# MeteoSwiss/topo-descriptors

Hardware: AMD Instinct MI355X
Metric: Mpixels/s (and % HBM roofline) per descriptor, 1/2/4/8 MI355X (higher is better)
Workload: dtype f32

## Files before the change

include/topo_amd.h:

```cpp
#ifndef TOPO_AMD_H
#define TOPO_AMD_H

#include <stddef.h>
#include <stdint.h>

#ifdef __cplusplus
extern "C" {
#endif

#define TOPO_AMD_OK 0
#define TOPO_AMD_EINVAL (-1)
#define TOPO_AMD_EHIP (-2)
#define TOPO_AMD_ENODEV (-3)
#define TOPO_AMD_ERCCL (-4)
#define TOPO_AMD_EUNSUP (-5)
#define TOPO_AMD_EEMPTY (-6)

#define TOPO_AMD_DESC_TPI 0
#define TOPO_AMD_DESC_STD 1
#define TOPO_AMD_DESC_GAUSS 2
#define TOPO_AMD_DESC_GRADIENT 3
#define TOPO_AMD_DESC_SOBEL 4
#define TOPO_AMD_DESC_SX 5
#define TOPO_AMD_DESC_VALLEY_RIDGE 6
// ... 44 lines not shown
int topo_amd_tpi_std_dev(const float* in, int in_rows, int in_row0, int gny, int nx, int size,
                         int out_row0, int out_rows, float* tpi_out, float* std_out);

int topo_amd_tpi_multi_dev(const float* in, int in_rows, int in_row0, int gny, int nx, int n_sizes,
                           const int32_t* sizes, int out_row0, int out_rows, float* const* tpi_outs);
int topo_amd_gaussian_dev(const float* in, int in_rows, int in_row0, int gny, int nx,
                          double sigma_y, double sigma_x, int out_row0, int out_rows,
                          float* out);

int topo_amd_sobel_dev(const float* in, int in_rows, int in_row0, int gny, int nx,
                       int out_row0, int out_rows, float* dx_out, float* dy_out);

int topo_amd_gradient_dev(const float* in, int in_rows, int in_row0, int gny, int nx,
                          double sigma, double sig_ratio, int res_mode, const void* res_x,
                          const void* res_y, int out_row0, int out_rows, float* dx_out,
                          float* dy_out, float* slope_out, float* aspect_out);

int topo_amd_sx_dev(const float* in, int in_rows, int in_row0, int gny, int nx,
                    const int32_t* dj, const int32_t* di, const double* dist, int n_off,
                    int window, double height, int out_row0, int out_rows, float* out);

int topo_amd_sx_multi_dev(const float* in, int in_rows, int in_row0, int gny, int nx, int n_az,
                          const int32_t* first, const int32_t* dj, const int32_t* di,
                          const double* dist, const int32_t* window, double height,
                          int out_row0, int out_rows, float* const* outs);

#define TOPO_AMD_VALLEY_MAX_PLANES 16
int topo_amd_valley_ridge_dev(const float* in, int in_rows, int in_row0, int gny, int nx,
                              const float* taps, const int32_t* ksize, const float* angles,
                              int n_angles, int n_planes, double mean, double stdev,
                              int out_row0, int out_rows, float* norm_out, float* dir_out);
int topo_amd_valley_route(int* route);
int topo_amd_tpi_route(int* route);
int topo_amd_mean_std_dev(const float* in, size_t count, double* mean, double* stdev);

int topo_amd_fill_na_dev(const float* in, int in_rows, int in_row0, int gny, int nx, const double* x_coords,
                         double min_elevation, int out_row0, int out_rows, float* out, uint8_t* missing_out);

int topo_amd_release_host_planes(void);
int topo_amd_host_chunks(int* chunks);
int topo_amd_tpi_f32(const float* dem, int ny, int nx, int size, double sigma, float* out);
int topo_amd_std_f32(const float* dem, int ny, int nx, int size, double sigma, float* out);
int topo_amd_tpi_std_f32(const float* dem, int ny, int nx, int size, double sigma,
                         float* tpi_out, float* std_out);
int topo_amd_tpi_std_multi_f32(const float* dem, int ny, int nx, int n_scales, const int32_t* sizes,
                               const double* sigmas, float* const* tpi_outs, float* const* std_outs);
int topo_amd_gauss_f32(const float* dem, int ny, int nx, double sigma_y, double sigma_x,
                       float* out);
int topo_amd_sobel_f32(const float* dem, int ny, int nx, float* dx_out, float* dy_out);
int topo_amd_fill_na_f32(const float* dem, int ny, int nx, const double* x_coords, double min_elevation, float* out,
                         uint8_t* missing_out);
int topo_amd_gradient_f32(const float* dem, int ny, int nx, double sigma, double sig_ratio,
                          int res_mode, const void* res_x, const void* res_y, float* dx_out,
                          float* dy_out, float* slope_out, float* aspect_out);
int topo_amd_sx_f32(const float* dem, int ny, int nx, const int32_t* dj, const int32_t* di,
                    const double* dist, int n_off, int window, double height, float* out);
int topo_amd_sx_multi_f32(const float* dem, int ny, int nx, int n_az, const int32_t* first,
                          const int32_t* dj, const int32_t* di, const double* dist,
                          const int32_t* window, double height, float* const* outs);
int topo_amd_valley_ridge_f32(const float* dem, int ny, int nx, const float* taps,
                              const int32_t* ksize, const float* angles, int n_angles,
                              int n_planes, double mean, double stdev, float* norm_out,
                              float* dir_out);

#define TOPO_AMD_F32 0
#define TOPO_AMD_I16 1
// ... 81 lines not shown
```

topo_descriptors_amd/_lib.py:

```python
import ctypes as C
import os
import threading

import numpy as np

HERE = os.path.dirname(os.path.abspath(__file__))
LIB_PATH = os.environ.get("TOPO_AMD_LIBRARY") or os.path.join(HERE, "libtopo_amd.so")

_f32p = C.POINTER(C.c_float)
_i32p = C.POINTER(C.c_int32)
_f64p = C.POINTER(C.c_double)
_vp = C.c_void_p


class Raster(C.Structure):
    _fields_ = [("data", C.c_void_p), ("dtype", C.c_int32), ("has_nodata", C.c_int32),
                ("scale", C.c_double), ("offset", C.c_double), ("nodata", C.c_double)]


_rp = C.POINTER(Raster)
F32, I16, U16, I32, U8, F64 = range(6)
SOURCE_DTYPES = {np.dtype(np.float32): F32, np.dtype(np.int16): I16, np.dtype(np.uint16): U16,
                 np.dtype(np.int32): I32, np.dtype(np.uint8): U8, np.dtype(np.float64): F64}

SIGNATURES = {
    "topo_amd_version": (C.c_char_p, []),
    "topo_amd_last_error": (C.c_char_p, []),
    "topo_amd_device_count": (C.c_int, []),
    "topo_amd_init": (C.c_int, [C.c_int]),
    "topo_amd_shutdown": (C.c_int, []),
    "topo_amd_device_name": (C.c_int, [C.c_char_p, C.c_int]),
    "topo_amd_malloc": (C.c_int, [C.POINTER(_vp), C.c_size_t]),
    "topo_amd_free": (C.c_int, [_vp]),
    "topo_amd_host_alloc": (C.c_int, [C.POINTER(C.c_void_p), C.c_size_t]),
    "topo_amd_host_free": (C.c_int, [C.c_void_p]),
    "topo_amd_memcpy_h2d": (C.c_int, [_vp, _vp, C.c_size_t]),
    "topo_amd_memcpy_d2h": (C.c_int, [_vp, _vp, C.c_size_t]),
    "topo_amd_memcpy_d2d": (C.c_int, [_vp, _vp, C.c_size_t]),
    "topo_amd_memset": (C.c_int, [_vp, C.c_int, C.c_size_t]),
    "topo_amd_sync": (C.c_int, []),
    "topo_amd_release_host_planes": (C.c_int, []),
    "topo_amd_host_chunks": (C.c_int, [_i32p]),
    "topo_amd_valley_route": (C.c_int, [_i32p]),
    "topo_amd_tpi_route": (C.c_int, [_i32p]),
    "topo_amd_dem_changed": (C.c_int, [_vp, C.c_size_t]),
    "topo_amd_raster_scan_dev": (C.c_int, [_vp, C.c_int, C.c_int, C.c_int, C.c_int, C.c_int, C.c_int,
                                           C.POINTER(C.c_uint64), _f32p]),
    "topo_amd_raster_class_from_scan": (C.c_int, [_vp, C.c_int, C.c_int, C.c_int, C.POINTER(C.c_uint64), _f32p]),
    "topo_amd_raster_class_set": (C.c_int, [_vp, C.c_int, C.c_int, C.c_int, C.c_int, C.c_float, C.c_float, C.c_float]),
    "topo_amd_raster_class_get": (C.c_int, [_vp, C.c_int, C.c_int, _i32p, _i32p, _f32p, _f32p, _f32p]),
    "topo_amd_shard_classify": (C.c_int, [_vp, C.c_int, C.c_int, C.c_int, C.c_int]),
    "topo_amd_timer_start": (C.c_int, []),
    "topo_amd_timer_stop": (C.c_int, [_f32p]),
    "topo_amd_mark": (C.c_int, [C.c_int]),
    "topo_amd_mark_elapsed": (C.c_int, [C.c_int, C.c_int, C.POINTER(C.c_float)]),
    "topo_amd_cu_count": (C.c_int, []),
    "topo_amd_synth_dem_dev": (C.c_int, [_vp, C.c_int, C.c_int, C.c_int, C.c_uint32, C.c_int]),
    "topo_amd_disc_tap_count": (C.c_int, [C.c_int]),
    "topo_amd_disc_mask": (C.c_int, [C.c_int, _f32p]),
    "topo_amd_halo_rows": (C.c_int, [C.c_int, C.c_double, C.c_double, _i32p, _i32p]),
    "topo_amd_tpi_std_dev": (C.c_int, [_vp, C.c_int, C.c_int, C.c_int, C.c_int, C.c_int, C.c_int,
                                       C.c_int, _vp, _vp]),
    "topo_amd_gaussian_dev": (C.c_int, [_vp, C.c_int, C.c_int, C.c_int, C.c_int, C.c_double,
                                        C.c_double, C.c_int, C.c_int, _vp]),
    "topo_amd_sobel_dev": (C.c_int, [_vp, C.c_int, C.c_int, C.c_int, C.c_int, C.c_int, C.c_int,
                                     _vp, _vp]),
    "topo_amd_gradient_dev": (C.c_int, [_vp, C.c_int, C.c_int, C.c_int, C.c_int, C.c_double,
                                        C.c_double, C.c_int, _vp, _vp, C.c_int, C.c_int, _vp, _vp,
                                        _vp, _vp]),
    "topo_amd_sx_dev": (C.c_int, [_vp, C.c_int, C.c_int, C.c_int, C.c_int, _i32p, _i32p, _f64p,
                                  C.c_int, C.c_int, C.c_double, C.c_int, C.c_int, _vp]),
    "topo_amd_tpi_multi_dev": (C.c_int, [_vp, C.c_int, C.c_int, C.c_int, C.c_int, C.c_int, _i32p, C.c_int, C.c_int,
                                         C.POINTER(_vp)]),
    "topo_amd_sx_multi_dev": (C.c_int, [_vp, C.c_int, C.c_int, C.c_int, C.c_int, C.c_int, _i32p, _i32p, _i32p,
                                        _f64p, _i32p, C.c_double, C.c_int, C.c_int, C.POINTER(_vp)]),
    "topo_amd_valley_ridge_dev": (C.c_int, [_vp, C.c_int, C.c_int, C.c_int, C.c_int, _vp, _i32p, _vp, C.c_int,
                                            C.c_int, C.c_double, C.c_double, C.c_int, C.c_int, _vp, _vp]),
# ... 160 lines not shown
```

topo_descriptors_amd/csrc/capi.hip:

```cpp
#include <rccl/rccl.h>

#include <algorithm>
#include <atomic>
#include <chrono>
#include <condition_variable>
#include <cmath>
#include <cstdio>
#include <cstdlib>
#include <cstring>
#include <map>
#include <mutex>

#include "common.hpp"
#include "decode.hpp"

#include <sys/mman.h>

#include <thread>

namespace topo {

static thread_local std::string g_error;

void set_error(const char* fmt, ...) {
// ... 940 lines not shown
    TOPO_REQUIRE(hptr != nullptr && bytes > 0, "host_alloc: bad arguments");
    TOPO_HIP(hipHostMalloc(hptr, bytes, hipHostMallocDefault));
    return TOPO_AMD_OK;
}
int topo_amd_host_free(void* hptr) {
    TOPO_ENTER();
    TOPO_TRY(require_ready());
    if (hptr) TOPO_HIP(hipHostFree(hptr));
    return TOPO_AMD_OK;
}

int topo_amd_release_host_planes(void) {
    TOPO_ENTER();
    TOPO_TRY(require_ready());
    Context& c = ctx();
    TOPO_HIP(hipStreamSynchronize(c.compute));
    for (size_t k = 0; k < c.host_planes.size(); ++k) {
        if (c.host_planes[k]) {
            dem_memo_forget(c.host_planes[k], c.host_plane_bytes[k]);
            TOPO_HIP(hipFree(c.host_planes[k]));
        }
    }
    c.host_planes.clear();
    c.host_plane_bytes.clear();
    return TOPO_AMD_OK;
}

int topo_amd_tpi_route(int* route) {
    TOPO_REQUIRE(route != nullptr, "tpi_route: NULL output");
    *route = t_tpi_route;
    return TOPO_AMD_OK;
}

int topo_amd_valley_route(int* route) {
    TOPO_REQUIRE(route != nullptr, "valley_route: NULL output");
    *route = t_valley_route;
    return TOPO_AMD_OK;
}

int topo_amd_host_chunks(int* chunks) {
    TOPO_REQUIRE(chunks != nullptr, "host_chunks: NULL output");
    *chunks = t_host_chunks;
    return TOPO_AMD_OK;
}

int topo_amd_memcpy_h2d(void* dst, const void* src, size_t bytes) {
    TOPO_ENTER();
    TOPO_TRY(require_ready());
    dem_memo_forget(dst, bytes);
    TOPO_HIP(hipMemcpyAsync(dst, src, bytes, hipMemcpyHostToDevice, ctx().compute));
    TOPO_HIP(hipStreamSynchronize(ctx().compute));
    return TOPO_AMD_OK;
}

int topo_amd_memcpy_d2h(void* dst, const void* src, size_t bytes) {
    TOPO_ENTER();
    TOPO_TRY(require_ready());
    {
        HostRun pages(false);
        pages.prefault(dst, bytes);
    }
    TOPO_HIP(hipMemcpyAsync(dst, src, bytes, hipMemcpyDeviceToHost, ctx().compute));
    TOPO_HIP(hipStreamSynchronize(ctx().compute));
    return check_gate_errors();
}

// ... 1215 lines not shown
    c.ghost = GhostGate();
    if (taken) return rc == TOPO_AMD_OK ? finish_gated(lean && device_gate, false) : rc;
    if (rc != TOPO_AMD_EUNSUP) return rc;
    return run_three(block, s, above, below, fn, true);
}


}
}

namespace {
int ensure_shard_class(const Shard& s) {
    if (s.rows_local == s.owned.gny || declared_class(s.owned, nullptr)) return TOPO_AMD_OK;
    return topo_amd_shard_classify(s.owned.in, s.rows_local, s.row0, s.owned.gny, s.owned.nx);
}
}

extern "C" {

int topo_amd_shard_tpi_std(float* block, int rows_local, int row0, int gny, int nx, int size,
                           float* tpi_out, float* std_out) {
    TOPO_ENTER();
    TOPO_TRY(require_ready());
    DiscRuns disc;
    TOPO_TRY(build_disc(size, &disc));
    const int above = -disc.dj_min, below = disc.dj_max;
    TOPO_TRY(shard_view(&block, above, below, "shard_tpi_std"));
    block += shard_view_offset(above, nx);
    Shard s = make_shard(block, rows_local, row0, gny, nx, above, below);
    TOPO_TRY(ensure_shard_class(s));
    ClassScope cls(s.owned);
    forget_plane(tpi_out, rows_local, nx);
    forget_plane(std_out, rows_local, nx);
    const int tile_rows = std_out ? std_tile_rows(size) : (size <= 17 ? 64 : 60);
    return run_fused(block, s, above, below, tile_rows, [&](const Block& view, int o0, int on) {
        Block b = view;
        b.out_row0 = o0;
        b.out_rows = on;
        TOPO_TRY(check_block(b, above, below, "shard_tpi_std"));
        return launch_tpi_std(b, disc, shift(tpi_out, o0 - row0, nx), shift(std_out, o0 - row0, nx));
    });
}

int topo_amd_shard_gradient(float* block, int rows_local, int row0, int gny, int nx, double sigma,
                            double sig_ratio, int res_mode, const void* res_x, const void* res_y,
                            float* dx_out, float* dy_out, float* slope_out, float* aspect_out) {
    TOPO_ENTER();
    TOPO_TRY(require_ready());
    const int h = gradient_ghost_rows(sigma, sig_ratio, false);
    TOPO_TRY(shard_view(&block, h, h, "shard_gradient"));
    block += shard_view_offset(h, nx);
    Shard s = make_shard(block, rows_local, row0, gny, nx, h, h);
    TOPO_TRY(ensure_shard_class(s));
    ClassScope cls(s.owned);
    for (float* o : {dx_out, dy_out, slope_out, aspect_out}) forget_plane(o, rows_local, nx);
    return run_gated(block, s, h, h, false, [&](const Block& view, int o0, int on) {
        Block b = view;
        b.out_row0 = o0;
        b.out_rows = on;
        TOPO_TRY(check_block(b, h, h, "shard_gradient"));
        const void *rx = res_x, *ry = res_y;
        if (res_mode == TOPO_AMD_RES_2D) {
            rx = (const float*)res_x + (size_t)(o0 - row0) * nx;
            ry = (const float*)res_y + (size_t)(o0 - row0) * nx;
        }
        return launch_gradient(b, sigma, sig_ratio, res_mode, rx, ry, shift(dx_out, o0 - row0, nx),
                               shift(dy_out, o0 - row0, nx), shift(slope_out, o0 - row0, nx),
// ... 255 lines not shown
```

topo_descriptors_amd/csrc/common.hpp:

```cpp
#pragma once

#include <hip/hip_runtime.h>

#include <cstdarg>
#include <cstdint>
#include <cstdio>
#include <mutex>
#include <string>
#include <vector>

#include "../../include/topo_amd.h"

namespace topo {

void set_error(const char* fmt, ...);

#define TOPO_HIP(call)                                                                     \
    do {                                                                                   \
        hipError_t e_ = (call);                                                            \
        if (e_ != hipSuccess) {                                                            \
            ::topo::set_error("%s failed: %s (%s:%d)", #call, hipGetErrorString(e_),       \
                              __FILE__, __LINE__);                                         \
            return TOPO_AMD_EHIP;                                                          \
        }                                                                                  \
// ... 22 lines not shown
constexpr size_t kGateBytes = 16384;
constexpr size_t kGateSlots = kGateBytes - 256;
struct Gate {
    const uint32_t* word;
    uint32_t epoch;
    uint32_t* timeouts;
    uint32_t limit_ticks;
    uint8_t* skipped;
    uint32_t* errors;
};

struct Seams {
    int n = 0;
    Block b[2];
    Gate gate{nullptr, 0, nullptr, 0, nullptr, nullptr};
    bool gate_armed = false;
};

struct GhostGate {
    bool armed = false;
    Gate gate{nullptr, 0, nullptr, 0, nullptr, nullptr};
    int ghost_lo = 0, ghost_hi = 0;
    size_t slots = 0;
};

constexpr int kWorkspaces = 15;
constexpr int kTables = 7;
struct Context {
    bool ready = false;
    int device = -1;
    int num_cu = 256;
    int reserve_cus = 0;
    Seams seams;
    GhostGate ghost;
    uint32_t* gate_word = nullptr;
    uint32_t* gate_timeouts = nullptr;
    uint32_t gate_epoch = 0;
    int gate_mode = 0;
    int gate_clean_calls = 0;
    hipEvent_t gate_probe = nullptr;
    bool gate_probe_pending = false;
    size_t lds_per_block = 65536;
    hipStream_t compute = nullptr;
    hipStream_t comm = nullptr;
    std::vector<void*> host_planes;
    std::vector<size_t> host_plane_bytes;
    hipStream_t up = nullptr, down = nullptr;
    std::vector<hipEvent_t> pipe_events;
    hipStream_t aux = nullptr;
    hipEvent_t aux_ready[64] = {};
    hipEvent_t aux_done = nullptr;
    hipEvent_t halo_done = nullptr;
    hipEvent_t input_ready = nullptr;
    hipEvent_t t0 = nullptr, t1 = nullptr;
    void* ws[kWorkspaces] = {};
    size_t ws_bytes[kWorkspaces] = {};
    void* tab[kTables] = {};
    size_t tab_bytes[kTables] = {};
};

Context& ctx();
int require_ready();

std::recursive_mutex& call_mutex();
struct CallGuard {
    std::lock_guard<std::recursive_mutex> lock;
    CallGuard();
    CallGuard(const CallGuard&) = delete;
    CallGuard& operator=(const CallGuard&) = delete;
};
#define TOPO_ENTER() ::topo::CallGuard call_guard_
int workspace(int slot, size_t bytes, void** out);
int upload_table(int slot, const void* host, size_t bytes, void** out);

int check_block(const Block& b, int need_above, int need_below, const char* who);
constexpr int kMaxLaunchRows = 65280;
inline int check_grid_rows(long rows, const char* who) {
    TOPO_REQUIRE(rows <= 65535, "%s: %ld rows in one call, the launch covers at most 65535 (gridDim.y): split the "
                 "request with out_row0 / out_rows", who, rows);
    return TOPO_AMD_OK;
}

struct DiscRuns {
    int size = 0;
    int taps = 0;
    int dj_min = 0, dj_max = 0;
    int di_min = 0, di_max = 0;
    int centre_dj = 0, centre_di = 0;
    std::vector<int16_t> lo, hi;
};
int build_disc(int size, DiscRuns* out);

int launch_tpi_std(const Block& b, const DiscRuns& disc, float* tpi_out, float* std_out);
int launch_disc_wave(const Block& b, int size, float* tpi_out, float* std_out);
bool disc_wave_covers(int size);
constexpr int kStdSpecMax = 41;
constexpr int std_tile_rows(int size) { return size >= 5 && size % 2 == 1 && size <= kStdSpecMax ? 48 : 60; }
int launch_tpi_pair(const Block& b, int size_a, float* out_a, int size_b, float* out_b);
bool tpi_pair_covers(int size_a, int size_b);
int launch_disc_big(const Block& b, const DiscRuns& disc, float* tpi_out, float* std_out);
int launch_gaussian(const Block& b, double sigma_y, double sigma_x, float* out);
int gauss_ghost_rows(double sigma);
int gradient_ghost_rows(double sigma, double sig_ratio, bool least);
int launch_sobel(const Block& b, float* dx_out, float* dy_out);
int launch_gradient(const Block& b, double sigma, double sig_ratio, int res_mode,
                    const void* res_x, const void* res_y, float* dx, float* dy, float* slope,
                    float* aspect);
int launch_sx(const Block& b, const int32_t* dj, const int32_t* di, const double* dist,
              int n_off, int window, double height, float* out);
int launch_sx_multi(const Block& b, int n_az, const int32_t* first, const int32_t* dj, const int32_t* di,
                    const double* dist, const int32_t* window, double height, float* const* outs);
int launch_synth(float* out, int rows, int row0, int nx, uint32_t seed, bool integer_valued);
int launch_fill_na(const Block& b, const double* xs, bool ascending, bool use_thresh, float thresh, float* out, uint8_t* missing);
struct VrGroup {
    int stride = 4;
    int p0 = 0;
    int n_live = 1;
    float floor = 0.0f;
    float mark = -1.0f;
};
int launch_valley_ridge_fft(const Block& b, const float* taps, int stride, const int32_t* ksize, const float* angles,
                            int n_angles, int n_planes, int kmax, double mean, double stdev, float* norm_out,
                            float* dir_out);
void valley_fft_release();
int valley_ridge_reach(const int32_t* ksize, int n_angles, int* above, int* below);
void note_tpi_route(int route);
void note_valley_route(int route);
constexpr int kValleyMfmaMaxKernel = 25;
constexpr int kValleyStreamMaxKernel = 120;
constexpr int kValleyMfmaTileRows = 32;
// ... 25 lines not shown
```

topo_descriptors_amd/csrc/disc.hip:

```cpp
#include "common.hpp"

#include <cstdlib>

namespace topo {

namespace {

constexpr int kThreads = 256;
constexpr int kTileW = 128;

struct DiscArgs {
    const float* in;
    float* tpi;
    float* sd;
    const int* runs;
    int in_rows, in_row0, gny, nx;
    int out_row0, out_rows;
    int tile_h;
    int n_disc_rows;
    int dj_min, di_min;
    int halo_cols;
    int centre_dj, centre_di;
    int taps;
};
// ... 298 lines not shown
            if (x + e < cols) d[e] = v[e];
    }
}

int repitch(const float* src, int src_pitch, float* dst, int dst_pitch, int width, int cols, int rows) {
    if (rows <= 0) return TOPO_AMD_OK;
    TOPO_TRY(check_grid_rows(rows, "disc (re-pitched copy)"));
    dim3 grid(((cols + 3) / 4 + kThreads - 1) / kThreads, rows);
    hipLaunchKernelGGL(repitch_kernel, grid, dim3(kThreads), 0, ctx().compute, src, src_pitch, dst, dst_pitch,
                       width, cols);
    TOPO_HIP(hipGetLastError());
    return TOPO_AMD_OK;
}

int launch_disc_wave_repitched(const Block& b, int size, float* tpi_out, float* std_out) {
    const int nxp = (b.nx + 3) & ~3;
    void *in_p = nullptr, *tpi_p = nullptr, *std_p = nullptr;
    TOPO_TRY(workspace(4, (size_t)b.in_rows * nxp * sizeof(float), &in_p));
    if (tpi_out) TOPO_TRY(workspace(5, (size_t)b.out_rows * nxp * sizeof(float), &tpi_p));
    if (std_out) TOPO_TRY(workspace(6, (size_t)b.out_rows * nxp * sizeof(float), &std_p));
    TOPO_TRY(repitch(b.in, b.nx, (float*)in_p, nxp, b.nx, nxp, b.in_rows));
    Block bp = b;
    bp.in = (const float*)in_p;
    bp.nx = nxp;
    const int r = launch_disc_wave(bp, size, (float*)tpi_p, (float*)std_p);
    if (r != TOPO_AMD_OK) return r;
    if (tpi_out) TOPO_TRY(repitch((const float*)tpi_p, nxp, tpi_out, b.nx, b.nx, b.nx, b.out_rows));
    if (std_out) TOPO_TRY(repitch((const float*)std_p, nxp, std_out, b.nx, b.nx, b.nx, b.out_rows));
    return TOPO_AMD_OK;
}

}

int launch_tpi_std(const Block& b, const DiscRuns& disc, float* tpi_out, float* std_out) {
    if (b.out_rows > kMaxLaunchRows) {
        ctx().seams.n = 0;
        for (int r = 0; r < b.out_rows; r += kMaxLaunchRows) {
            Block s = b;
            s.out_row0 = b.out_row0 + r;
            s.out_rows = std::min(kMaxLaunchRows, b.out_rows - r);
            TOPO_TRY(launch_tpi_std(s, disc, tpi_out ? tpi_out + (size_t)r * b.nx : nullptr, std_out ? std_out + (size_t)r * b.nx : nullptr));
        }
        return TOPO_AMD_OK;
    }
    TOPO_REQUIRE(tpi_out || std_out, "tpi_std: both outputs are NULL");
    Context& c = ctx();
    if (c.seams.n > 0 && !(disc_wave_covers(disc.size) && b.nx % 4 == 0 && (reinterpret_cast<uintptr_t>(b.in) & 15) == 0 &&
                           (reinterpret_cast<uintptr_t>(std_out) & 15) == 0 && (reinterpret_cast<uintptr_t>(tpi_out) & 15) == 0))
        c.seams.n = 0;
    note_tpi_route(0);
    {
        int r = launch_disc_wave(b, disc.size, tpi_out, std_out);
        if (r == TOPO_AMD_EUNSUP && disc_wave_covers(disc.size) && b.nx >= 4)
            r = launch_disc_wave_repitched(b, disc.size, tpi_out, std_out);
        if (r != TOPO_AMD_EUNSUP) return r;
    }
    constexpr int big_from = 70;
    if (disc.size >= big_from) return launch_disc_big(b, disc, tpi_out, std_out);
    const int n_rows = disc.dj_max - disc.dj_min + 1;
    const int halo_cols = disc.di_max - disc.di_min;
    const int cols_v = kTileW + halo_cols;
    const int stride = (cols_v + 1) | 1;
    int tile_h = 32;
    auto lds_for = [&](int th) { return (size_t)(th + n_rows - 1) * stride * sizeof(float); };
    const size_t lds_cap = 160 * 1024;
    while (tile_h > 8 && lds_for(tile_h) > lds_cap) tile_h /= 2;
// ... 44 lines not shown
```

topo_descriptors_amd/csrc/disc_ring_wide_impl.hpp:

```cpp
#pragma once

namespace topo {

namespace {

constexpr int NCW = 6;

template <int SIZE>
struct WGeo {
    static constexpr DiscTable<SIZE> T = make_disc_table<SIZE>();
    static_assert(T.centre == 0 && T.off_min == -T.off_max, "odd disc sizes only");
    static constexpr int M = T.off_max;
    static constexpr int DL = (M + NCW - 1) / NCW;
    static constexpr int NVL = 64 - 2 * DL;
    static constexpr int TILE_W = NCW * NVL;
    static constexpr int X0 = NCW * DL;
    static constexpr int W = 64 * NCW;
    static constexpr int NR = T.num_runs;
    static_assert(NVL >= 16, "disc too wide for one wavefront");
    struct Sched {
        int first_step[SIZE];
        int order[SIZE];
        int centre_run;
    };
// ... 251 lines not shown
            for (int w = 0; w < 2; ++w) {
                cv[w] = row[PT::T.use[j][w][0]][s / 2][s % 2] - row[PT::T.use[j][w][1]][s / 2][s % 2];
                if (r == G::S.centre_run) ctr[w][s] = cv[w];
            }
            wide_static_for<(DL + 1) * NCW>([&](auto ET) {
                constexpr int E = decltype(ET)::value / NCW, t = decltype(ET)::value % NCW;
                constexpr int dr = NCW * E + s - t, dl = -NCW * E + s - t;
                if constexpr (dr >= 0 && dr <= M) {
                    if constexpr (G::T.run_of[dr - G::T.off_min] == r) {
                        static_assert(E <= D, "a run arrives at the first step that takes it");
#pragma unroll
                        for (int w = 0; w < 2; ++w) pR[w][E][t] = SW_::T.firstR[E][t] == j * NCW + s ? cv[w] : pR[w][E][t] + cv[w];
                    }
                }
                if constexpr (dl < 0 && dl >= -M) {
                    if constexpr (G::T.run_of[dl - G::T.off_min] == r) {
                        static_assert(E <= D, "a run arrives at the first step that takes it");
#pragma unroll
                        for (int w = 0; w < 2; ++w) pL[w][E][t] = SW_::T.firstL[E][t] == j * NCW + s ? cv[w] : pL[w][E][t] + cv[w];
                    }
                }
            });
        });
        RING_SB();
        wide_static_for<D - Dnext>([&](auto C) { close(std::integral_constant<int, D - decltype(C)::value>{}); });
    });
#pragma unroll
    for (int w = 0; w < 2; ++w)
#pragma unroll
        for (int t = 0; t < NCW; ++t) acc[w][t] = aR[w][t];
}


template <int SIZE>
__global__ __launch_bounds__(WideCfg<SIZE>::NW * 64) void tpi_ring_wide_kernel(WaveArgs p, int tiles_x, int tiles_y, PartRun deal) {
    using G = WGeo<SIZE>;
    using C = WideCfg<SIZE>;
    constexpr int B = C::B, R = C::R, PPT = C::PPT, SW = C::SW, NB_PRO = C::NB_PRO, DL = G::DL;
    constexpr unsigned kWindow = (1u << NB_PRO) - 1u;
    constexpr int kBad = 1, kFracOnly = 1 << 15;
    constexpr unsigned kHistMask = kWindow | kWindow * kFracOnly;
    extern __shared__ __attribute__((aligned(16))) uint32_t lds_u[];
    uint32_t* Q = lds_u;
    int* wflags = reinterpret_cast<int*>(Q + (R + C::GR) * G::W);

    const int nb = (int)gridDim.x;
    const int vb = (nb & 7) ? (int)blockIdx.x : (int)(blockIdx.x & 7) * (nb >> 3) + (int)(blockIdx.x >> 3);
    const int lane = threadIdx.x & 63;
    const int wave = __builtin_amdgcn_readfirstlane((int)(threadIdx.x >> 6));
    const int ntiles = tiles_x * tiles_y;
    const int first = deal.first(vb);
    const int last = min(first + deal.count(vb), ntiles);
    const double inv_nm1 = 1.0 / ((double)G::T.taps - 1.0);
    const int rmin = max(0, p.in_row0), rmax = min(p.gny, p.in_row0 + p.in_rows);
    const bool stager = wave < SW;
    const int scol = 128 * wave + 2 * lane;
    int seen_tiles = 0, seen_frac = 0;

#pragma unroll 1
    for (int pos = first; pos < last;) {
        const int tile0 = pos;
        const int ty0 = tile0 % tiles_y;
        const int run_tiles = min(last - tile0, tiles_y - ty0);
        const int strip = tile0 / tiles_y;
        const int nphase = run_tiles * PPT;
        const int ox0 = strip * G::TILE_W;
        const int oyS = (p.out_row0 / C::TH + ty0) * C::TH;
        const int gx0 = ox0 - G::X0;
        const int gy0 = oyS - G::M - C::PAD;
        const int gcol = gx0 + scol;
        const bool col_ok = stager && gcol >= 0 && gcol < p.nx;
        const float* src = p.in + (col_ok ? gcol : 0);
        auto load_batch = [&](int n0, float2 (&v)[B]) {
#pragma unroll
            for (int r = 0; r < B; ++r) {
                int gy = gy0 + n0 + r;
                gy = min(max(gy, rmin), rmax - 1);
                v[r] = *reinterpret_cast<const float2*>(src + (size_t)(gy - p.in_row0) * p.nx);
            }
        };
        uint32_t run0 = 0, run1 = 0;
        int wslot = 0;
// ... 42 lines not shown
        __syncthreads();
        auto run_phases = [&](auto STG) {
        constexpr bool stg = decltype(STG)::value;
        float2 va[stg ? B : 1];
        if constexpr (stg) {
            int bits = 0;
#pragma unroll 1
            for (int k = 0; k < NB_PRO; ++k) {
                load_batch(k * B, va);
                bits |= stage_batch(k * B, va) << (NB_PRO - 1 - k);
                advance_wslot();
            }
            if (lane == 0) wflags[wave] = bits;
            load_batch(C::PRO, va);
        } else {
            for (int k = 0; k < NB_PRO; ++k) advance_wslot();
        }
        __syncthreads();
        {
            int all = 0;
#pragma unroll
            for (int w = 0; w < SW; ++w) all |= wflags[w];
            hist = (unsigned)__builtin_amdgcn_readfirstlane(all) & kHistMask;
        }

        bool tile_frac = false;
#pragma unroll 1
        for (int ph = 0; ph < nphase; ++ph) {
            const bool compute = (hist & kWindow) == 0;
            const int oyA = oyS + ph * B;
            tile_frac = tile_frac || (hist & (kWindow * kFracOnly)) != 0;
            if (!compute) {
                const int r0 = max(oyA, p.out_row0), r1 = min(oyA + B, p.out_row0 + p.out_rows) - 1;
                if (r0 <= r1 && threadIdx.x == 0) {
                    const int base = p.out_row0 / p.map_th;
                    const int mx0 = ox0 / p.map_tw, mx1 = (min(ox0 + G::TILE_W, p.nx) - 1) / p.map_tw;
                    for (int mx = mx0; mx <= mx1; ++mx)
                        for (int my = r0 / p.map_th; my <= r1 / p.map_th; ++my) p.defer[mx * p.map_tiles_y + (my - base)] = kNeedsFraction;
                }
            }
            if (ph % PPT == PPT - 1) {
                ++seen_tiles;
                seen_frac += tile_frac ? 1 : 0;
                tile_frac = false;
            }
            if constexpr (stg) {
                const int seen = stage_batch(C::PRO + ph * B, va);
                if (lane == 0) wflags[((ph + 1) & 1) * SW + wave] = seen;
                load_batch(C::PRO + (ph + 1) * B, va);
            } else if (compute) {
                static_assert(C::RPW == 2, "a chain wave sums its two rows of a phase in one sweep");
                const int j = (wave - SW) * C::RPW;
                const int oy = oyA + j;
                if (oy + C::RPW > p.out_row0 && oy < p.out_row0 + p.out_rows) {
                    const int s0 = (C::PAD - 1 + ph * B + j) % R;
                    uint32_t acc[C::RPW][NCW], ctr[C::RPW][NCW];
                    wide_pair_sum<SIZE, R, C::GR, WIDE_LEAD, WIDE_PRIO != 0>(Q, s0, lane, acc, ctr);
#pragma unroll
                    for (int k = 0; k < C::RPW; ++k) {
                        const bool row_ok = oy + k >= p.out_row0 && oy + k < p.out_row0 + p.out_rows;
                        if (lane_ok && row_ok) {
                            float* o = p.tpi + (size_t)(oy + k - p.out_row0) * p.nx + ocol;
                            float out_t[NCW];
#pragma unroll
                            for (int t = 0; t < NCW; ++t) {
                                const int xi = (int)ctr[k][t];
                                out_t[t] = (float)((double)xi - (double)((int)acc[k][t] - xi) * inv_nm1);
                            }
#pragma unroll
                            for (int P = 0; P < NCW / 2; ++P)
                                if (ocol + 2 * P < p.nx) *reinterpret_cast<float2*>(o + 2 * P) = make_float2(out_t[2 * P], out_t[2 * P + 1]);
                        }
                    }
                }
            }
            advance_wslot();
            __syncthreads();
            fold((ph + 1) & 1);
        }
        };
        if (stager) run_phases(std::true_type{});
        else run_phases(std::false_type{});
        pos += run_tiles;
    }
    if (p.report != nullptr && vb == nb / 2 && threadIdx.x == 0) {
        __hip_atomic_store(p.report + 1, (uint32_t)seen_frac, __ATOMIC_RELAXED, __HIP_MEMORY_SCOPE_SYSTEM);
        __hip_atomic_store(p.report, (uint32_t)seen_tiles, __ATOMIC_RELAXED, __HIP_MEMORY_SCOPE_SYSTEM);
    }
}

template <int SIZE>
int launch_ring_wide(const Block& b, float* tpi_out, int map_th, int map_tw) {
    using G = WGeo<SIZE>;
    using C = WideCfg<SIZE>;
    Context& c = ctx();
    TOPO_REQUIRE(c.seams.n == 0, "the wide ring takes single-block calls only");
    WaveArgs a{b.in, tpi_out, nullptr, b.in_rows, b.in_row0, b.gny, b.nx, b.out_row0, b.out_rows,
               nullptr, nullptr, nullptr, 0, 0, 0};
    static int blocks_per_cu = 0;
    if (blocks_per_cu == 0) {
        TOPO_HIP(hipFuncSetAttribute((const void*)tpi_ring_wide_kernel<SIZE>, hipFuncAttributeMaxDynamicSharedMemorySize, (int)C::LDS));
        int nblk = 0;
        TOPO_HIP(hipOccupancyMaxActiveBlocksPerMultiprocessor(&nblk, (const void*)tpi_ring_wide_kernel<SIZE>, C::NW * 64, C::LDS));
        blocks_per_cu = nblk < 1 ? 1 : nblk;
    }
    a.report = dem_memo_report(b);
    WaveParts ps;
    int tiles_x = 0;
    long ntiles = 0;
    TOPO_TRY(make_parts(b, a, C::TH, G::TILE_W, true, false, &ps, &tiles_x, &ntiles, map_th, map_tw));
    TOPO_REQUIRE(ps.n == 1 && ps.a[0].map_th == map_th && ps.a[0].map_tw == map_tw, "wide ring: tile map of another geometry");
    const size_t map_bytes = (size_t)((b.nx + map_tw - 1) / map_tw) * ps.a[0].map_tiles_y;
    TOPO_HIP(hipMemsetAsync(ps.a[0].defer, kTileDone, map_bytes, c.compute));
    const long grid = march_grid(c, blocks_per_cu, ntiles);
    deal_parts(&ps, tiles_x, grid, blocks_per_cu);
    hipLaunchKernelGGL(tpi_ring_wide_kernel<SIZE>, dim3((unsigned)grid), dim3(C::NW * 64), C::LDS, c.compute, ps.a[0], tiles_x, ps.tiles_y[0], ps.run[0]);
    TOPO_HIP(hipGetLastError());
    return TOPO_AMD_OK;
}

}

}
```

topo_descriptors_amd/csrc/disc_wave_impl.hpp:

```cpp
#pragma once
#include <algorithm>
#include <cmath>
#include <cstdlib>
#include <type_traits>

#include "common.hpp"
#include "disc_runs.hpp"
#include "gate.hpp"

namespace topo {

namespace {

constexpr int NC = 4;
constexpr int ROWW = 64 * NC;

constexpr int cdiv_floor(int a, int b) { return (a >= 0) ? a / b : -((-a + b - 1) / b); }
constexpr int cdiv_ceil(int a, int b) { return -cdiv_floor(-a, b); }

template <int SIZE>
struct Geo {
    static constexpr DiscTable<SIZE> T = make_disc_table<SIZE>();
    static constexpr int D_LO = cdiv_ceil(T.off_min - (NC - 1), NC);
    static constexpr int D_HI = cdiv_floor(T.off_max + (NC - 1), NC);
// ... 1818 lines not shown
    TOPO_TRY(workspace(2, (size_t)grid * kScratchPlanes * TH * ROWW * sizeof(uint32_t), &scratch));
    for (int k = 0; k < kMaxParts; ++k) ps.a[k].scratch = (uint32_t*)scratch;
    deal_parts(&ps, tiles_x, grid, blocks_per_cu);
    return launch_parts(nullptr, disc_wave_kernel<SIZE, TH, NWAVES, WANT_TPI, WANT_STD>, grid, NWAVES * 64, lds, ps, tiles_x);
}

}

}

#include "disc_ring_impl.hpp"
#include "disc_ring_wide_impl.hpp"

namespace topo {

namespace {

constexpr int tile_rows(int size, int nwaves, int cap) {
    int th = cap;
    while (th > nwaves && (size_t)(th + size + nwaves) * ROWW * 4 + (size_t)(th * (size + 1) + 8) * 2 + 16 > 160 * 1024)
        th -= nwaves;
    return th;
}

inline int env_int(const char* name, int fallback) {
    const char* e = std::getenv(name);
    return e ? std::atoi(e) : fallback;
}
constexpr int std_march_min_size() { return 31; }
constexpr int tpi_march_min_size() { return 1; }
constexpr int tpi_ring_min_size() { return 5; }
constexpr int std_ring_min_size() { return 5; }
constexpr int tpi_ring_max_size() { return 17; }
constexpr int tpi_wide_min_size() { return 67; }
constexpr int tpi_wide_max_size() { return 67; }
inline bool tpi_wide_ring() {
    static const int v = env_int("TOPO_AMD_TPI_WIDE_RING", 1);
    return v != 0;
}
inline bool tpi_fraction_scaled() {
    static const int v = env_int("TOPO_AMD_TPI_FRACTION_EXACT", 0);
    return v == 0;
}
constexpr int tpi_fraction_min_size() { return 17; }
inline bool std_spec_wide() {
    static const int v = env_int("TOPO_AMD_STD_SPEC_WIDE", 1);
    return v != 0;
}

template <int SIZE>
int launch_wave_any(const Block& b, float* tpi_out, float* std_out) {
    constexpr int TH8 = tile_rows(SIZE, 8, 64), TH12 = tile_rows(SIZE, 12, 60);
    constexpr bool kFullTile = TH12 == 60;
    if constexpr (std_ring_fits(SIZE) && !std_ring_both_fits(SIZE) && kFullTile) {
        if (std_out && current_class().frac_share > 0.5f) {
            if (tpi_out) TOPO_TRY((launch_march_sums<SIZE, TH12, 12, true>(b, tpi_out)));
            else TOPO_TRY((launch_march_sums<SIZE, TH12, 12, false>(b, nullptr)));
            TOPO_TRY((launch_std_march<SIZE, TH12, 12, true>(b, std_out)));
            TOPO_TRY((launch_fraction_march<SIZE, TH12, 12, true>(b, tpi_out, std_out)));
            if (tpi_out) return launch_wave<SIZE, TH8, 8, true, true>(b, tpi_out, std_out, true, TH12);
            return launch_wave<SIZE, TH8, 8, false, true>(b, tpi_out, std_out, true, TH12);
        }
    }
    if constexpr (std_ring_fits(SIZE)) {
        if (std_out && SIZE >= std_ring_min_size()) {
            if constexpr (std_spec_wide_fits(SIZE)) {
                const bool big = (long)b.nx * b.out_rows >= (1L << 27);
                if (current_class().frac_share == 0.0f && std_spec_wide() && (tpi_out != nullptr || (SIZE <= 7 && big))) {
                    if (tpi_out) TOPO_TRY((launch_std_ring_spec<SIZE, true, false, 8>(b, tpi_out, std_out)));
                    else TOPO_TRY((launch_std_ring_spec<SIZE, false, false, 8>(b, nullptr, std_out)));
                    if (tpi_out) return launch_wave<SIZE, TH8, 8, true, true>(b, tpi_out, std_out, true, StdRingCfg<SIZE>::TH, RGeo<SIZE, 8>::TILE_W);
                    return launch_wave<SIZE, TH8, 8, false, true>(b, tpi_out, std_out, true, StdRingCfg<SIZE>::TH, RGeo<SIZE, 8>::TILE_W);
                }
            }
            if constexpr (std_ring_spec(SIZE)) {
                if (tpi_out) TOPO_TRY((launch_std_ring_spec<SIZE, true>(b, tpi_out, std_out)));
// ... 14 lines not shown
            if (tpi_out) return launch_wave<SIZE, TH8, 8, true, true>(b, tpi_out, std_out, true, StdRingCfg<SIZE>::TH);
            return launch_wave<SIZE, TH8, 8, false, true>(b, tpi_out, std_out, true, StdRingCfg<SIZE>::TH);
        }
    }
    if (std_out && (SIZE < std_march_min_size() || !kFullTile)) {
        if (tpi_out) return launch_wave<SIZE, TH8, 8, true, true>(b, tpi_out, std_out);
        return launch_wave<SIZE, TH8, 8, false, true>(b, tpi_out, std_out);
    }
    if (std_out) {
        if (tpi_out) {
            TOPO_TRY((launch_march<SIZE, TH12, 12, true, true>(b, tpi_out)));
        } else {
            TOPO_TRY((launch_march<SIZE, TH12, 12, false, true>(b, nullptr)));
        }
        TOPO_TRY((launch_std_march<SIZE, TH12, 12>(b, std_out)));
        if (tpi_out) return launch_wave<SIZE, TH8, 8, true, true>(b, tpi_out, std_out, true, TH12);
        return launch_wave<SIZE, TH8, 8, false, true>(b, tpi_out, std_out, true, TH12);
    }
    if (SIZE < tpi_march_min_size()) return launch_wave<SIZE, TH12, 12, true, false>(b, tpi_out, std_out);
    constexpr bool kRing = ring_both_fits(SIZE) && SIZE <= 17;
    if constexpr (kRing) {
        if (SIZE >= tpi_ring_min_size() && SIZE <= tpi_ring_max_size()) {
            using RC = RingCfg<SIZE, 8>;
            constexpr int map_tw = RGeo<SIZE, 8>::TILE_W;
            TOPO_TRY((launch_ring<SIZE, 8, kRingMark>(b, tpi_out)));
            TOPO_TRY((launch_ring<SIZE, 8, kRingBoth>(b, tpi_out)));
            return launch_wave<SIZE, TH12, 12, true, false>(b, tpi_out, std_out, true, RC::TH, map_tw);
        }
    }
    if (SIZE < tpi_fraction_min_size()) {
        TOPO_TRY((launch_march<SIZE, TH12, 12, true, false, false>(b, tpi_out)));
        return launch_wave<SIZE, TH12, 12, true, false>(b, tpi_out, std_out, true);
    }
    if constexpr (tpi_wide_ring_fits(SIZE) && SIZE >= tpi_wide_min_size() && SIZE <= tpi_wide_max_size()) {
        const bool one_block = b.out_row0 == 0 && b.out_rows == b.gny && ctx().seams.n == 0;
        if (tpi_wide_ring() && tpi_fraction_scaled() && one_block && current_class().frac_share == 0.0f &&
            !dem_memo_mostly_fractional(b)) {
            TOPO_TRY((launch_ring_wide<SIZE>(b, tpi_out, TH12, Geo<SIZE>::TILE_W)));
            note_tpi_route(1);
            TOPO_TRY((launch_scaled_march<SIZE, TH12, 12>(b, tpi_out)));
            return launch_wave<SIZE, TH12, 12, true, false>(b, tpi_out, std_out, true);
        }
    }
    if (tpi_fraction_scaled()) {
        if (dem_memo_mostly_fractional(b) || current_class().frac_share > 0.5f) {
            TOPO_TRY((launch_scaled_march<SIZE, TH12, 12, true>(b, tpi_out)));
            return launch_wave<SIZE, TH12, 12, true, false>(b, tpi_out, std_out, true);
        }
        TOPO_TRY((launch_march<SIZE, TH12, 12, true, true, true>(b, tpi_out, true)));
        TOPO_TRY((launch_scaled_march<SIZE, TH12, 12>(b, tpi_out)));
        return launch_wave<SIZE, TH12, 12, true, false>(b, tpi_out, std_out, true);
    }
    TOPO_TRY((launch_march<SIZE, TH12, 12, true, true, true>(b, tpi_out)));
    TOPO_TRY((launch_fraction_march<SIZE, TH12, 12>(b, tpi_out)));
    return launch_wave<SIZE, TH12, 12, true, false>(b, tpi_out, std_out, true);
}

}

}
```

topo_descriptors_amd/csrc/gate.hpp:

```cpp
#pragma once
#include <hip/hip_runtime.h>

#include "common.hpp"

namespace topo {

__device__ __forceinline__ bool gate_wait(const Gate& g, const unsigned slot) {
    if (g.word == nullptr) return true;
    uint8_t* mine = g.skipped + slot;
    if (threadIdx.x == 0) {
        const long long t0 = __builtin_amdgcn_s_memtime();
        uint8_t gave_up = 0;
        while ((int)(__hip_atomic_load(g.word, __ATOMIC_RELAXED, __HIP_MEMORY_SCOPE_SYSTEM) - g.epoch) < 0) {
            if ((unsigned long long)(__builtin_amdgcn_s_memtime() - t0) > (unsigned long long)g.limit_ticks) {
                __hip_atomic_fetch_add(g.errors ? g.errors : g.timeouts, 1u, __ATOMIC_RELAXED, __HIP_MEMORY_SCOPE_SYSTEM);
                gave_up = 1;
                break;
            }
            __builtin_amdgcn_s_sleep(16);
        }
        __hip_atomic_store(mine, gave_up, __ATOMIC_RELAXED, __HIP_MEMORY_SCOPE_WORKGROUP);
    }
    __syncthreads();
    const bool open = __hip_atomic_load(mine, __ATOMIC_RELAXED, __HIP_MEMORY_SCOPE_WORKGROUP) == 0;
    __builtin_amdgcn_fence(__ATOMIC_ACQUIRE, "");
    return open;
}

}
```

Before: 315,300.

## Route sharded size-67 TPI through the wide ring kernel with multi-part launches

Extends the wide-ring TPI path, previously restricted to single-block calls, to sharded multi-device calls. The ring kernel gains a multi-part variant that walks several parts behind a gate, and the sharded entry point now picks 64-row tiles aligned to the wide ring geometry. The intent is to avoid the slower march fallback on sharded runs at size 67. The cost is extra routing state in the context, gate waiting between parts, and a requirement that the parts' tile maps sit contiguously in memory.

Measured after the change: 314,400. About the same (-0.3%).

```diff
diff --git a/include/topo_amd.h b/include/topo_amd.h
--- a/include/topo_amd.h
+++ b/include/topo_amd.h
@@ -100,6 +100,8 @@
                               int out_row0, int out_rows, float* norm_out, float* dir_out);
 int topo_amd_valley_route(int* route);
 int topo_amd_tpi_route(int* route);
+int topo_amd_tpi_route_plan(int size, int want_tpi, int want_std, float frac_share, int mostly_fractional, int one_block,
+                            int sharded, int* wide, int* shard_tile_rows);
 int topo_amd_mean_std_dev(const float* in, size_t count, double* mean, double* stdev);
 
 int topo_amd_fill_na_dev(const float* in, int in_rows, int in_row0, int gny, int nx, const double* x_coords,
diff --git a/topo_descriptors_amd/_lib.py b/topo_descriptors_amd/_lib.py
--- a/topo_descriptors_amd/_lib.py
+++ b/topo_descriptors_amd/_lib.py
@@ -43,6 +43,7 @@
     "topo_amd_host_chunks": (C.c_int, [_i32p]),
     "topo_amd_valley_route": (C.c_int, [_i32p]),
     "topo_amd_tpi_route": (C.c_int, [_i32p]),
+    "topo_amd_tpi_route_plan": (C.c_int, [C.c_int, C.c_int, C.c_int, C.c_float, C.c_int, C.c_int, C.c_int, _i32p, _i32p]),
     "topo_amd_dem_changed": (C.c_int, [_vp, C.c_size_t]),
     "topo_amd_raster_scan_dev": (C.c_int, [_vp, C.c_int, C.c_int, C.c_int, C.c_int, C.c_int, C.c_int,
                                            C.POINTER(C.c_uint64), _f32p]),
diff --git a/topo_descriptors_amd/csrc/capi.hip b/topo_descriptors_amd/csrc/capi.hip
--- a/topo_descriptors_amd/csrc/capi.hip
+++ b/topo_descriptors_amd/csrc/capi.hip
@@ -996,6 +996,15 @@
     return TOPO_AMD_OK;
 }
 
+int topo_amd_tpi_route_plan(int size, int want_tpi, int want_std, float frac_share, int mostly_fractional, int one_block,
+                            int sharded, int* wide, int* shard_tile_rows) {
+    TOPO_REQUIRE(wide != nullptr && shard_tile_rows != nullptr, "tpi_route_plan: NULL output");
+    const bool w = tpi_wide_candidate(size, want_tpi != 0, want_std != 0, frac_share, mostly_fractional != 0, one_block != 0, sharded != 0);
+    *wide = w ? 1 : 0;
+    *shard_tile_rows = shard_tpi_std_tile_rows(size, want_std != 0, w);
+    return TOPO_AMD_OK;
+}
+
 int topo_amd_valley_route(int* route) {
     TOPO_REQUIRE(route != nullptr, "valley_route: NULL output");
     *route = t_valley_route;
@@ -2277,7 +2286,15 @@
     ClassScope cls(s.owned);
     forget_plane(tpi_out, rows_local, nx);
     forget_plane(std_out, rows_local, nx);
-    const int tile_rows = std_out ? std_tile_rows(size) : (size <= 17 ? 64 : 60);
+    struct ShardedTpi {
+        ShardedTpi() { ctx().sharded_tpi = true; }
+        ~ShardedTpi() { ctx().sharded_tpi = false; }
+    } sharded;
+    Block owned_rows = s.owned;
+    owned_rows.out_row0 = row0;
+    owned_rows.out_rows = rows_local;
+    const bool wide = tpi_wide_route(owned_rows, size, tpi_out != nullptr, std_out != nullptr);
+    const int tile_rows = shard_tpi_std_tile_rows(size, std_out != nullptr, wide);
     return run_fused(block, s, above, below, tile_rows, [&](const Block& view, int o0, int on) {
         Block b = view;
         b.out_row0 = o0;
diff --git a/topo_descriptors_amd/csrc/common.hpp b/topo_descriptors_amd/csrc/common.hpp
--- a/topo_descriptors_amd/csrc/common.hpp
+++ b/topo_descriptors_amd/csrc/common.hpp
@@ -78,6 +78,7 @@
     int num_cu = 256;
     int reserve_cus = 0;
     Seams seams;
+    bool sharded_tpi = false;
     GhostGate ghost;
     uint32_t* gate_word = nullptr;
     uint32_t* gate_timeouts = nullptr;
@@ -142,6 +143,13 @@
 bool disc_wave_covers(int size);
 constexpr int kStdSpecMax = 41;
 constexpr int std_tile_rows(int size) { return size >= 5 && size % 2 == 1 && size <= kStdSpecMax ? 48 : 60; }
+constexpr int kTpiWideMinSize = 67, kTpiWideMaxSize = 67;
+constexpr int kTpiWideTileRows = 64;
+bool tpi_wide_ring();
+bool tpi_fraction_scaled();
+bool tpi_wide_candidate(int size, bool want_tpi, bool want_std, float frac_share, bool mostly_fractional, bool one_block, bool sharded);
+bool tpi_wide_route(const Block& b, int size, bool want_tpi, bool want_std);
+int shard_tpi_std_tile_rows(int size, bool want_std, bool wide);
 int launch_tpi_pair(const Block& b, int size_a, float* out_a, int size_b, float* out_b);
 bool tpi_pair_covers(int size_a, int size_b);
 int launch_disc_big(const Block& b, const DiscRuns& disc, float* tpi_out, float* std_out);
diff --git a/topo_descriptors_amd/csrc/disc.hip b/topo_descriptors_amd/csrc/disc.hip
--- a/topo_descriptors_amd/csrc/disc.hip
+++ b/topo_descriptors_amd/csrc/disc.hip
@@ -354,6 +354,33 @@
 
 }
 
+bool tpi_wide_ring() {
+    static const bool on = [] {
+        const char* e = std::getenv("TOPO_AMD_TPI_WIDE_RING");
+        return !(e && std::atoi(e) == 0);
+    }();
+    return on;
+}
+bool tpi_fraction_scaled() {
+    static const bool on = [] {
+        const char* e = std::getenv("TOPO_AMD_TPI_FRACTION_EXACT");
+        return !(e && std::atoi(e) != 0);
+    }();
+    return on;
+}
+bool tpi_wide_candidate(int size, bool want_tpi, bool want_std, float frac_share, bool mostly_fractional, bool one_block, bool sharded) {
+    return size >= kTpiWideMinSize && size <= kTpiWideMaxSize && size % 2 == 1 && want_tpi && !want_std && tpi_wide_ring() &&
+           tpi_fraction_scaled() && frac_share == 0.0f && !mostly_fractional && (one_block || sharded);
+}
+bool tpi_wide_route(const Block& b, int size, bool want_tpi, bool want_std) {
+    const Context& c = ctx();
+    const bool one_block = b.out_row0 == 0 && b.out_rows == b.gny && c.seams.n == 0;
+    return tpi_wide_candidate(size, want_tpi, want_std, current_class().frac_share, dem_memo_mostly_fractional(b), one_block, c.sharded_tpi);
+}
+int shard_tpi_std_tile_rows(int size, bool want_std, bool wide) {
+    return want_std ? std_tile_rows(size) : (size <= 17 || wide ? kTpiWideTileRows : 60);
+}
+
 int launch_tpi_std(const Block& b, const DiscRuns& disc, float* tpi_out, float* std_out) {
     if (b.out_rows > kMaxLaunchRows) {
         ctx().seams.n = 0;
diff --git a/topo_descriptors_amd/csrc/disc_ring_wide_impl.hpp b/topo_descriptors_amd/csrc/disc_ring_wide_impl.hpp
--- a/topo_descriptors_amd/csrc/disc_ring_wide_impl.hpp
+++ b/topo_descriptors_amd/csrc/disc_ring_wide_impl.hpp
@@ -307,8 +307,9 @@
 }
 
 
-template <int SIZE>
-__global__ __launch_bounds__(WideCfg<SIZE>::NW * 64) void tpi_ring_wide_kernel(WaveArgs p, int tiles_x, int tiles_y, PartRun deal) {
+template <int SIZE, bool PARTS>
+__device__ __forceinline__ void tpi_ring_wide_body(const WaveArgs& p, int tiles_x, int tiles_y, const PartRun deal, const int vb0, const int nb,
+                                                   const int tid) {
     using G = WGeo<SIZE>;
     using C = WideCfg<SIZE>;
     constexpr int B = C::B, R = C::R, PPT = C::PPT, SW = C::SW, NB_PRO = C::NB_PRO, DL = G::DL;
@@ -319,10 +320,9 @@
     uint32_t* Q = lds_u;
     int* wflags = reinterpret_cast<int*>(Q + (R + C::GR) * G::W);
 
-    const int nb = (int)gridDim.x;
-    const int vb = (nb & 7) ? (int)blockIdx.x : (int)(blockIdx.x & 7) * (nb >> 3) + (int)(blockIdx.x >> 3);
-    const int lane = threadIdx.x & 63;
-    const int wave = __builtin_amdgcn_readfirstlane((int)(threadIdx.x >> 6));
+    const int vb = PARTS ? (vb0 + deal.shift) % nb : vb0;
+    const int lane = tid & 63;
+    const int wave = __builtin_amdgcn_readfirstlane((int)(tid >> 6));
     const int ntiles = tiles_x * tiles_y;
     const int first = deal.first(vb);
     const int last = min(first + deal.count(vb), ntiles);
@@ -431,7 +431,7 @@
             tile_frac = tile_frac || (hist & (kWindow * kFracOnly)) != 0;
             if (!compute) {
                 const int r0 = max(oyA, p.out_row0), r1 = min(oyA + B, p.out_row0 + p.out_rows) - 1;
-                if (r0 <= r1 && threadIdx.x == 0) {
+                if (r0 <= r1 && tid == 0) {
                     const int base = p.out_row0 / p.map_th;
                     const int mx0 = ox0 / p.map_tw, mx1 = (min(ox0 + G::TILE_W, p.nx) - 1) / p.map_tw;
                     for (int mx = mx0; mx <= mx1; ++mx)
@@ -482,9 +482,41 @@
         else run_phases(std::false_type{});
         pos += run_tiles;
     }
-    if (p.report != nullptr && vb == nb / 2 && threadIdx.x == 0) {
+    if (p.report != nullptr && vb == nb / 2 && tid == 0) {
         __hip_atomic_store(p.report + 1, (uint32_t)seen_frac, __ATOMIC_RELAXED, __HIP_MEMORY_SCOPE_SYSTEM);
         __hip_atomic_store(p.report, (uint32_t)seen_tiles, __ATOMIC_RELAXED, __HIP_MEMORY_SCOPE_SYSTEM);
+    }
+}
+
+template <int SIZE>
+__global__ __launch_bounds__(WideCfg<SIZE>::NW * 64) void tpi_ring_wide_kernel(WaveArgs p, int tiles_x, int tiles_y, PartRun deal) {
+    const int nb = (int)gridDim.x;
+    const int vb = (nb & 7) ? (int)blockIdx.x : (int)(blockIdx.x & 7) * (nb >> 3) + (int)(blockIdx.x >> 3);
+    tpi_ring_wide_body<SIZE, false>(p, tiles_x, tiles_y, deal, vb, nb, (int)threadIdx.x);
+}
+
+template <int SIZE>
+__global__ __launch_bounds__(WideCfg<SIZE>::NW * 64) void tpi_ring_wide_kernel_parts(WaveParts ps, int tiles_x) {
+    const int nb = (int)gridDim.x;
+    const int vb = (nb & 7) ? (int)blockIdx.x : (int)(blockIdx.x & 7) * (nb >> 3) + (int)(blockIdx.x >> 3);
+    const int wave_s = __builtin_amdgcn_readfirstlane((int)(threadIdx.x >> 6));
+    auto thread_now = [&]() {
+        uint32_t all = ~0u;
+        asm volatile("" : "+s"(all));
+        return wave_s * 64 + (int)__builtin_amdgcn_mbcnt_hi(all, __builtin_amdgcn_mbcnt_lo(all, 0u));
+    };
+    if (ps.cleanup) {
+        if (ps.gate.skipped[blockIdx.x] == 0) return;
+        __syncthreads();
+        if (thread_now() == 0) ps.gate.skipped[blockIdx.x] = 0;
+    } else {
+        tpi_ring_wide_body<SIZE, false>(ps.a[0], tiles_x, ps.tiles_y[0], ps.run[0], vb, nb, thread_now());
+        if (!gate_wait(ps.gate, blockIdx.x, thread_now()) && ps.gate.errors == nullptr) return;
+    }
+#pragma unroll 1
+    for (int part = 1; part < ps.n; ++part) {
+        __syncthreads();
+        tpi_ring_wide_body<SIZE, true>(ps.a[part], tiles_x, ps.tiles_y[part], ps.run[part], vb, nb, thread_now());
     }
 }
 
@@ -493,7 +525,6 @@
     using G = WGeo<SIZE>;
     using C = WideCfg<SIZE>;
     Context& c = ctx();
-    TOPO_REQUIRE(c.seams.n == 0, "the wide ring takes single-block calls only");
     WaveArgs a{b.in, tpi_out, nullptr, b.in_rows, b.in_row0, b.gny, b.nx, b.out_row0, b.out_rows,
                nullptr, nullptr, nullptr, 0, 0, 0};
     static int blocks_per_cu = 0;
@@ -508,16 +539,18 @@
     int tiles_x = 0;
     long ntiles = 0;
     TOPO_TRY(make_parts(b, a, C::TH, G::TILE_W, true, false, &ps, &tiles_x, &ntiles, map_th, map_tw));
-    TOPO_REQUIRE(ps.n == 1 && ps.a[0].map_th == map_th && ps.a[0].map_tw == map_tw, "wide ring: tile map of another geometry");
-    const size_t map_bytes = (size_t)((b.nx + map_tw - 1) / map_tw) * ps.a[0].map_tiles_y;
+    size_t map_bytes = 0;
+    for (int k = 0; k < ps.n; ++k) {
+        TOPO_REQUIRE(ps.a[k].map_th == map_th && ps.a[k].map_tw == map_tw, "wide ring: tile map of another geometry");
+        TOPO_REQUIRE(ps.a[k].defer == ps.a[0].defer + map_bytes, "wide ring: the parts' tile maps are not contiguous");
+        map_bytes += (size_t)((b.nx + map_tw - 1) / map_tw) * ps.a[k].map_tiles_y;
+    }
     TOPO_HIP(hipMemsetAsync(ps.a[0].defer, kTileDone, map_bytes, c.compute));
     const long grid = march_grid(c, blocks_per_cu, ntiles);
     deal_parts(&ps, tiles_x, grid, blocks_per_cu);
-    hipLaunchKernelGGL(tpi_ring_wide_kernel<SIZE>, dim3((unsigned)grid), dim3(C::NW * 64), C::LDS, c.compute, ps.a[0], tiles_x, ps.tiles_y[0], ps.run[0]);
-    TOPO_HIP(hipGetLastError());
-    return TOPO_AMD_OK;
-}
-
-}
-
-}
+    return launch_parts(tpi_ring_wide_kernel<SIZE>, tpi_ring_wide_kernel_parts<SIZE>, grid, C::NW * 64, C::LDS, ps, tiles_x);
+}
+
+}
+
+}
diff --git a/topo_descriptors_amd/csrc/disc_wave_impl.hpp b/topo_descriptors_amd/csrc/disc_wave_impl.hpp
--- a/topo_descriptors_amd/csrc/disc_wave_impl.hpp
+++ b/topo_descriptors_amd/csrc/disc_wave_impl.hpp
@@ -1874,16 +1874,6 @@
 constexpr int tpi_ring_min_size() { return 5; }
 constexpr int std_ring_min_size() { return 5; }
 constexpr int tpi_ring_max_size() { return 17; }
-constexpr int tpi_wide_min_size() { return 67; }
-constexpr int tpi_wide_max_size() { return 67; }
-inline bool tpi_wide_ring() {
-    static const int v = env_int("TOPO_AMD_TPI_WIDE_RING", 1);
-    return v != 0;
-}
-inline bool tpi_fraction_scaled() {
-    static const int v = env_int("TOPO_AMD_TPI_FRACTION_EXACT", 0);
-    return v == 0;
-}
 constexpr int tpi_fraction_min_size() { return 17; }
 inline bool std_spec_wide() {
     static const int v = env_int("TOPO_AMD_STD_SPEC_WIDE", 1);
@@ -1964,10 +1954,9 @@
         TOPO_TRY((launch_march<SIZE, TH12, 12, true, false, false>(b, tpi_out)));
         return launch_wave<SIZE, TH12, 12, true, false>(b, tpi_out, std_out, true);
     }
-    if constexpr (tpi_wide_ring_fits(SIZE) && SIZE >= tpi_wide_min_size() && SIZE <= tpi_wide_max_size()) {
-        const bool one_block = b.out_row0 == 0 && b.out_rows == b.gny && ctx().seams.n == 0;
-        if (tpi_wide_ring() && tpi_fraction_scaled() && one_block && current_class().frac_share == 0.0f &&
-            !dem_memo_mostly_fractional(b)) {
+    if constexpr (tpi_wide_ring_fits(SIZE) && SIZE >= kTpiWideMinSize && SIZE <= kTpiWideMaxSize) {
+        static_assert(WideCfg<SIZE>::TH == kTpiWideTileRows, "the sharded entry point aligns its seams to these tile rows");
+        if (tpi_wide_route(b, SIZE, tpi_out != nullptr, std_out != nullptr)) {
             TOPO_TRY((launch_ring_wide<SIZE>(b, tpi_out, TH12, Geo<SIZE>::TILE_W)));
             note_tpi_route(1);
             TOPO_TRY((launch_scaled_march<SIZE, TH12, 12>(b, tpi_out)));
diff --git a/topo_descriptors_amd/csrc/gate.hpp b/topo_descriptors_amd/csrc/gate.hpp
--- a/topo_descriptors_amd/csrc/gate.hpp
+++ b/topo_descriptors_amd/csrc/gate.hpp
@@ -5,10 +5,10 @@
 
 namespace topo {
 
-__device__ __forceinline__ bool gate_wait(const Gate& g, const unsigned slot) {
+__device__ __forceinline__ bool gate_wait(const Gate& g, const unsigned slot, const int tid) {
     if (g.word == nullptr) return true;
     uint8_t* mine = g.skipped + slot;
-    if (threadIdx.x == 0) {
+    if (tid == 0) {
         const long long t0 = __builtin_amdgcn_s_memtime();
         uint8_t gave_up = 0;
         while ((int)(__hip_atomic_load(g.word, __ATOMIC_RELAXED, __HIP_MEMORY_SCOPE_SYSTEM) - g.epoch) < 0) {
@@ -26,5 +26,6 @@
     __builtin_amdgcn_fence(__ATOMIC_ACQUIRE, "");
     return open;
 }
+__device__ __forceinline__ bool gate_wait(const Gate& g, const unsigned slot) { return gate_wait(g, slot, (int)threadIdx.x); }
 
 }
```
